# RemoteSensingTools/vSmartMOM.jl

Hardware: AMD Instinct MI355X
Metric: spectral-points/s (whole node) for rt_run, O2-A band (higher is better)
Workload: dtype f64; 1 GPU; C2: O2-A 759-770 nm, nStokes=3, Nquad=20 (N=60), 40 layers, 10000 spectral points/GPU, m=0..2, Rayleigh+synthetic O2 absorption, Lambertian 0.15; ranks=1, collective_backend=none (1 rank), N=60, layers=40, points_per_gpu=10000, fourier_moments=3

## Files before the change

include/vsmartmom_hip.h:

```cpp
#ifndef VSMARTMOM_HIP_H
#define VSMARTMOM_HIP_H

#include <stddef.h>
#include <stdint.h>

#ifdef __cplusplus
extern "C" {
#endif

typedef enum vsm_status {
  VSM_OK = 0,
  VSM_ERR_INVALID_ARG = 1,
  VSM_ERR_UNSUPPORTED = 2,
  VSM_ERR_HIP = 3,
  VSM_ERR_NO_DEVICE = 4
} vsm_status;

typedef enum vsm_iface {
  VSM_IFACE_00 = 0,
  VSM_IFACE_01 = 1,
  VSM_IFACE_10 = 2,
  VSM_IFACE_11 = 3
} vsm_iface;

// ... 387 lines not shown
int vsm_run_create_view_f64(const vsm_quad_f64* q, int S, int nm, const int* m_h, const int* coupling_h, void* workspace,
                            size_t workspace_bytes, unsigned flags, int nrows, const int* rows_h, vsm_run** run);
int vsm_run_create_view_f32(const vsm_quad_f32* q, int S, int nm, const int* m_h, const int* coupling_h, void* workspace,
                            size_t workspace_bytes, unsigned flags, int nrows, const int* rows_h, vsm_run** run);
int vsm_run_layer_f64(vsm_run* run, int ndoubl, const double* dtau, const double* varpi, const double* tau_sum,
                      const double* F0, int ncomp, const double* const* Zpp, const double* const* Zmp, long long z_stride,
                      const double* fcomp, int toa, const int* layer_coupling_h, void* stream);
int vsm_run_layer_f32(vsm_run* run, int ndoubl, const float* dtau, const float* varpi, const float* tau_sum,
                      const float* F0, int ncomp, const float* const* Zpp, const float* const* Zmp, long long z_stride,
                      const float* fcomp, int toa, const int* layer_coupling_h, void* stream);
int vsm_run_export_f64(vsm_run* run, const vsm_composite_f64* comps, void* stream);
int vsm_run_export_f32(vsm_run* run, const vsm_composite_f32* comps, void* stream);
int vsm_run_import_f64(vsm_run* run, const vsm_composite_f64* comps, void* stream);
int vsm_run_import_f32(vsm_run* run, const vsm_composite_f32* comps, void* stream);
int vsm_run_zw_tail(vsm_run* run);
int vsm_run_view_rows(vsm_run* run, int nrows, const int* rows_h);
int vsm_run_view_block(const vsm_run* run, int block, int* im, int* n, int* nv, int* local_rows);
int vsm_run_view_rows(vsm_run* run, int nrows, const int* rows_h);
int vsm_run_view_block(const vsm_run* run, int block, int* im, int* n, int* nv, int* local_rows);
int vsm_run_destroy(vsm_run* run);
enum { VSM_SURFACE_LAMBERTIAN_SCALAR = 0, VSM_SURFACE_LAMBERTIAN_SPECTRAL = 1, VSM_SURFACE_BRDF = 2 };
enum { VSM_SURFACE_LAYER_IDENTITY = 1 };
unsigned vsm_surface_layer_flags(int kind, int m, int has_surface_source);
int vsm_run_export_moment_f64(vsm_run* run, int im, const vsm_composite_f64* comp, void* stream);
int vsm_run_export_moment_f32(vsm_run* run, int im, const vsm_composite_f32* comp, void* stream);
int vsm_run_export_sources_f64(vsm_run* run, int im, const vsm_composite_f64* comp, void* stream);
int vsm_run_export_sources_f32(vsm_run* run, int im, const vsm_composite_f32* comp, void* stream);
int vsm_run_surface_f64(vsm_run* run, int im, int iface, const vsm_added_f64* added_surface, int identity, int matrices,
                        const vsm_composite_f64* comp, double* work, void* stream);
int vsm_run_surface_f32(vsm_run* run, int im, int iface, const vsm_added_f32* added_surface, int identity, int matrices,
                        const vsm_composite_f32* comp, float* work, void* stream);
int vsm_run_guard_once(vsm_run* run);
int vsm_run_counters(const vsm_run* run, int* counts_h);
int vsm_stokes_coupling_f64(int N, int n_stokes, int nblocks, const double* Zpp, const double* Zmp, int* mask_d, void* stream);
int vsm_stokes_coupling_f32(int N, int n_stokes, int nblocks, const float* Zpp, const float* Zmp, int* mask_d, void* stream);

typedef struct vsm_added_rs_f64 {
  double *ier_mp, *iet_pp, *ier_pm, *iet_mm;
  double *ieJ0_p, *ieJ0_m;
  int K;
  int reserved;
} vsm_added_rs_f64;
typedef struct vsm_added_rs_f32 {
  float *ier_mp, *iet_pp, *ier_pm, *iet_mm;
  float *ieJ0_p, *ieJ0_m;
  int K;
  int reserved;
} vsm_added_rs_f32;
typedef struct vsm_composite_rs_f64 {
  double *ieR_mp, *ieR_pm, *ieT_pp, *ieT_mm;
  double *ieJ0_p, *ieJ0_m;
  int K;
  int reserved;
} vsm_composite_rs_f64;
typedef struct vsm_composite_rs_f32 {
  float *ieR_mp, *ieR_pm, *ieT_pp, *ieT_mm;
  float *ieJ0_p, *ieJ0_m;
  int K;
  int reserved;
} vsm_composite_rs_f32;
typedef struct vsm_rrs_f64 {
  const int* shift;
  const double* varpi_ie;
  const double* fscatt;
  const double* Zpp;
  const double* Zmp;
// ... 272 lines not shown
```

vsmartmom.jl_amd/_lib.py:

```python
from __future__ import annotations

import ctypes as C
import os

_HERE = os.path.dirname(os.path.abspath(__file__))
LIB_PATH = os.environ.get("VSM_LIB_PATH") or os.path.join(_HERE, "lib", "libvsmartmom_hip.so")


class VSMError(RuntimeError):
    pass


class vsm_quad_f64(C.Structure):
    _fields_ = [("mu", C.c_void_p), ("wt", C.c_void_p), ("N", C.c_int), ("n_stokes", C.c_int),
                ("i_mu0", C.c_int), ("mu0", C.c_double)]


class vsm_quad_f32(C.Structure):
    _fields_ = [("mu", C.c_void_p), ("wt", C.c_void_p), ("N", C.c_int), ("n_stokes", C.c_int),
                ("i_mu0", C.c_int), ("mu0", C.c_float)]


class vsm_added(C.Structure):
    _fields_ = [("r_mp", C.c_void_p), ("t_pp", C.c_void_p), ("r_pm", C.c_void_p), ("t_mm", C.c_void_p),
# ... 115 lines not shown
    "vsm_interaction_inelastic_rrs_{T}": (_I, [_I, _I, _I, _P, _P, _P, _P, _P, _P, _P]),
    "vsm_copy_added_to_composite_ie_{T}": (_I, [_I, _I, _P, _P, _P]),
    "vsm_postprocess_vza_ie_{T}": (_I, [_I, _I, _I, _I, _I, _P, _P, _P, _P, _P, _P, _P]),
    "vsm_ss_column_{T}": (_I, [_P, _I, _I, _I, _P, _P, _P, _P, _P, _P, _P, _P, _P, _P, _I, _P, _P, _P, _P, _P, _P, _P]),
    "vsm_ss_column_lin_{T}": (_I, [_P, _I, _I, _I, _I, _I, _I, _I, _I, _P, _P, _P, _P, _P, _P, _P, _P, _P, _P, _I, _P, _P, _P, _P, _P, _P, _P,
                                   _P, _P, _I, _P, _P, _P, _P, _P]),
    "vsm_ss_column_rrs_{T}": (_I, [_P, _I, _I, _I, _I, _P, _P, _P, _P, _P, _P, _P, _P, _I, _I, _P, _P, _P, _P, _P]),
    "vsm_ss_column_rrs_lin_{T}": (_I, [_P, _I, _I, _I, _I, _I, _I, _I, _I, _P, _P, _P, _P, _P, _P, _P, _P, _P, _P, _P, _I, _I, _P, _P, _P,
                                       _P, _P]),
    "vsm_exact_ss_path1_{T}": (_I, [_I, _I, _I, _I, _I, _P, _P, _P, _P, "{R}", _P, _P, _P]),
    "vsm_exact_ss_path2_{T}": (_I, [_I, _I, _I, _I, _I, _P, _P, _I, _P, "{R}", _P, _P, _P]),
    "vsm_exact_ss_path34_{T}": (_I, [_I, _I, _I, _I, _I, _P, _P, _P, _P, _P, _P, _P, _P, "{R}", _P, _P, _P, _P]),
    "vsm_exact_ss_jac12_{T}": (_I, [_I, _I, _I, _I, _I, _P, _P, _P, _P, _I, _P, "{R}", _P, _P, _P, _P, _P, _P, _P]),
    "vsm_run_supported": (_I, [_I, _I, _I]),
    "vsm_run_workspace_bytes": (_SZ, [_I, _I, _I, _I, _P]),
    "vsm_run_supported_f32": (_I, [_I, _I, _I]),
    "vsm_run_workspace_bytes_f32": (_SZ, [_I, _I, _I, _I, _P]),
    "vsm_run_create_{T}": (_I, [_P, _I, _I, _P, _P, _P, _SZ, _P]),
    "vsm_run_create_ex_{T}": (_I, [_P, _I, _I, _P, _P, _P, _SZ, C.c_uint, _P]),
    "vsm_run_create_view_{T}": (_I, [_P, _I, _I, _P, _P, _P, _SZ, C.c_uint, _I, _P, _P]),
    "vsm_run_layer_{T}": (_I, [_P, _I, _P, _P, _P, _P, _I, _P, _P, _LL, _P, _I, _P, _P]),
    "vsm_run_export_{T}": (_I, [_P, _P, _P]),
    "vsm_run_import_{T}": (_I, [_P, _P, _P]),
    "vsm_run_zw_tail": (_I, [_P]),
    "vsm_run_view_rows": (_I, [_P, _I, _P]),
    "vsm_run_view_block": (_I, [_P, _I, _P, _P, _P, _P]),
    "vsm_run_destroy": (_I, [_P]),
    "vsm_surface_layer_flags": (C.c_uint, [_I, _I, _I]),
    "vsm_run_export_moment_{T}": (_I, [_P, _I, _P, _P]),
    "vsm_run_export_sources_{T}": (_I, [_P, _I, _P, _P]),
    "vsm_run_surface_{T}": (_I, [_P, _I, _I, _P, _I, _I, _P, _P, _P]),
    "vsm_run_guard_once": (_I, [_P]),
    "vsm_run_counters": (_I, [_P, _P]),
    "vsm_stokes_coupling_{T}": (_I, [_I, _I, _I, _P, _P, _P, _P]),
    "vsm_level_radiance_work_elems": (_SZ, [_I, _I]),
    "vsm_level_radiance_{T}": (_I, [_I, _I, _I, _I, _P, _P, _P, _P, _P, _LL, _P, _P, _P, _P, _P, _P, _P]),
    "vsm_level_radiance_oplevel_{T}": (_I, [_I, _I, _I, _I, _P, _P, _P, _P, _P, _LL, _P, _P, _P, _P, _P, _P, _P]),
    "vsm_level_radiance_src_{T}": (_I, [_I, _I, _I, _I, _P, _P, _P, _I, _P, _P, _LL, _P, _P, _P, _P, _P, _P, _P]),
    "vsm_level_flux_{T}": (_I, [_I, _I, _I, _P, _I, _P, _P, _LL, _P, _I, _P, _P, "{R}", _P, _P, _P, _P]),
    "vsm_surface_emission_response_{T}": (_I, [_I, _I, _I, _I, _P, _I, _P, _P, _P, _P, _P, _LL, _P, _P, _P]),
    "vsm_level_radiance_ie_{T}": (_I, [_I, _I, _I, _I, _P, _I, _P, _P, _P, _P, _LL, _P, _P, _P, _P, _P, _P, _P, _P, _P, _P, _P]),
    "vsm_level_flux_ie_{T}": (_I, [_I, _I, _I, _I, _P, _P, _P, _LL, _P, _P, _P, _P, _P, _P, _I, _P, _P, "{R}", _P, _P, _P, _P]),
    "vsm_level_radiance_lin_{T}": (_I, [_I, _I, _I, _I, _I, _I, _P, _P, _P, _P, _LL, _P, _P, _P, _LL, _P, _P, _LL, _LL, _P, _P, _P, _P, _P,
                                        _P]),
    "vsm_level_radiance_lin_src_{T}": (_I, [_I, _I, _I, _I, _I, _I, _I, _P, _P, _P, _P, _LL, _P, _P, _P, _LL, _P, _P, _LL, _LL, _P, _P, _P,
                                            _P, _P, _P, _P, _P]),
    "vsm_level_flux_lin_{T}": (_I, [_I, _I, _I, _I, _I, _I, _P, _P, _LL, _P, _P, _P, _LL, _P, _P, _LL, _LL, _P, _P, _P, _I, _P, _P,
                                    "{R}", _P, _P, _P, _I, _P, _P]),
    "vsm_mie_work_elems": (_SZ, [_I, _I, _I]),
    "vsm_mie_nai2": (_I, [_I, _I, _I, C.c_double, C.c_double, C.c_double, _P, _P, _P, _P, _P, _P, _P, _P, _P, _P, _P]),
    "vsm_mie_lin_work_elems": (_SZ, [_I, _I, _I]),
    "vsm_mie_nai2_lin": (_I, [_I, _I, _I, C.c_double, C.c_double, C.c_double] + [_P] * 16),
    "vsm_dbge_work_elems": (_SZ, [_I, _I]),
    "vsm_truncate_dbge": (_I, [_I, _I, _I, C.c_double, _P, _P, _P, _P, _P, _P, _P, _P, _P, _P]),
    "vsm_dbge_lin_work_elems": (_SZ, [_I, _I]),
    "vsm_truncate_dbge_lin": (_I, [_I, _I, _I, C.c_double] + [_P] * 15),
    "vsm_absorption_chunk": (_I, []),
    "vsm_absorption_work_elems": (_SZ, [_I, _I]),
    "vsm_absorption_xsec": (_I, [_I, _I, _I, _I] + [_P] * 15 + [C.c_double, C.c_double, _I, _I, _I, _P, _P, _P]),
    "vsm_absorption_lin_chunk": (_I, []),
    "vsm_absorption_lin_work_elems": (_SZ, [_I, _I]),
    "vsm_absorption_xsec_lin": (_I, [_I, _I, _I, _I] + [_P] * 16 + [C.c_double, C.c_double, _I, _I, _I] + [_P] * 6),
    "vsm_absorption_profile_slots": (_I, [_I, _I, _I] + [_P] * 6),
    "vsm_test_lds_mm_{T}": (_I, [_I, _I, _P, _P, _P, _P]),
    "vsm_test_lds_inv_{T}": (_I, [_I, _I, _P, _P, _I, _P, _P]),
    "vsm_test_poison_lds": (_I, [_P]),
# ... 97 lines not shown
```

vsmartmom.jl_amd/core_rt.py:

```python
from __future__ import annotations

import contextlib
import ctypes as C
import dataclasses
import math
import os
import warnings
from dataclasses import dataclass
from typing import List, Optional

import numpy as np
import torch

from . import _lib
from . import host_model as H
from .architectures import GPU, CPU, architecture, array_type, devi, synchronize_if_gpu, to_host

IFACE = {"00": 0, "01": 1, "10": 2, "11": 3}
MOMENT_BATCH = 4
MOMENT_BATCH_MAX = 24
MOMENT_BATCHING = True
THERMAL_FUSION = True
NATIVE_RUN = True
NATIVE_SOURCES_ONLY = True
NATIVE_VIEW_ROWS = True
VIEW_ROWS_MAX = 16
NATIVE_ZW_TAIL = True
NATIVE_IDENTITY_SURFACE = True
NATIVE_DROPIN = True
REFERENCE_ORDER = False


def _require_gpu(arch):
    if not isinstance(arch, GPU):
        raise _lib.VSMError("vsmartmom.jl_amd provides the MI355X path only; architecture %r has no compute path here "
                            "(no CPU fallback by design)" % (arch,))
    if not torch.cuda.is_available():
        raise _lib.VSMError("no MI355X visible to HIP (torch.cuda.is_available() is False)")
    if arch.device_index != torch.cuda.current_device():
        raise _lib.VSMError("architecture GPU(%d) is not the current HIP device (%d): one process per GPU -- call "
                            "torch.cuda.set_device(%d) first" % (arch.device_index, torch.cuda.current_device(),
                                                                 arch.device_index))


def _torch_dtype(FT):
    return torch.float64 if np.dtype(FT) == np.float64 else torch.float32


def _stream_ptr():
    return C.c_void_p(torch.cuda.current_stream().cuda_stream)


def _ptr(t: Optional[torch.Tensor]):
    return C.c_void_p(0 if t is None else t.data_ptr())


def to_device_matrix(A: np.ndarray, arch, FT) -> torch.Tensor:
    A = np.asarray(A, dtype=FT)
    if A.ndim == 2:
        A = A[None]
# ... 68 lines not shown
    def __init__(self, FT, arch, N, nSpec, shared=False, d_symmetric=0):
        dev, dt = devi(arch), _torch_dtype(FT)
        sm = 1 if shared else nSpec
        z = lambda: torch.zeros((sm, N, N), dtype=dt, device=dev)
        self.r_mp, self.t_pp = z(), z()
        self.d_symmetric = int(d_symmetric)
        self.r_pm, self.t_mm = (None, None) if self.d_symmetric else (z(), z())
        self.j0_p = torch.zeros((nSpec, N), dtype=dt, device=dev)
        self.j0_m = torch.zeros((nSpec, N), dtype=dt, device=dev)
        self.N, self.nSpec, self.shared, self.dtype = N, nSpec, shared, dt

    def cstruct(self):
        return _lib.vsm_added(self.r_mp.data_ptr(), self.t_pp.data_ptr(),
                              0 if self.r_pm is None else self.r_pm.data_ptr(),
                              0 if self.t_mm is None else self.t_mm.data_ptr(),
                              self.j0_p.data_ptr(), self.j0_m.data_ptr(), 0 if self.shared else self.N * self.N,
                              self.d_symmetric, 0)


def _composite_field(name):
    vector = name in ("J0_p", "J0_m")

    def fget(self):
        if vector and self._vectors_current:
            return self._arr[name]
        return self.materialize()._arr[name]

    def fset(self, value):
        self.materialize()._arr[name] = value
    return property(fget, fset)


RUN_COUNTERS = ("exports_full", "exports_src", "surface_interactions", "guard_launches")


class RunRef:

    def __init__(self, run, sink=None, keep=None, refs: int = 1):
        self.run, self.sink, self.keep, self.refs = run, sink, keep, refs

    def release(self):
        self.refs -= 1
        if self.refs == 0 and self.run is not None:
            run, self.run = self.run, None
            L = _lib.lib()
            if self.sink is not None:
                counts = (C.c_int * 4)()
                if L.vsm_run_counters(run, counts) == 0:
                    for k, v in zip(RUN_COUNTERS, counts):
                        self.sink[k] = self.sink.get(k, 0) + int(v)
            L.vsm_run_destroy(run)
            self.keep = None


class CompositeLayer:

    def __init__(self, FT, arch, N, nSpec):
        dev, dt = devi(arch), _torch_dtype(FT)
        z = lambda: torch.zeros((nSpec, N, N), dtype=dt, device=dev)
        self._native = None
        self._sources_only = False
        self._view_rows = None
        self._native_ws = None
        self._vectors_current = False
        self._counters = None
        self._arr = dict(R_mp=z(), R_pm=z(), T_pp=z(), T_mm=z(), J0_p=torch.zeros((nSpec, N), dtype=dt, device=dev),
                         J0_m=torch.zeros((nSpec, N), dtype=dt, device=dev))
        self.N, self.nSpec, self.dtype = N, nSpec, dt

    R_mp, R_pm, T_pp = _composite_field("R_mp"), _composite_field("R_pm"), _composite_field("T_pp")
    T_mm, J0_p, J0_m = _composite_field("T_mm"), _composite_field("J0_p"), _composite_field("J0_m")

    def materialize(self):
        slot = self._native
        if slot is None:
            return self
        self._native, self._vectors_current = None, False
        try:
            cc = self._cstruct_raw()
            _lib.call("vsm_run_export_moment", self.dtype, slot.run, slot.im, C.byref(cc), _stream_ptr())
        finally:
            slot.ref.release()
        return self
# ... 785 lines not shown
                    m = mom["m"]
                    weight = float(fourier_weight(FT, m))
                    flags = create_surface_layer_(model.surface, self.added_surface, m, self.dq, mom["tau_sum_surface"], rho=mom["rho"],
                                                  has_surface_source=has_surface_source)
                    if surface_source_contribute_(self, model.surface, self.added_surface, m):
                        flags &= ~SURFACE_LAYER_IDENTITY
                    identity = bool(flags & SURFACE_LAYER_IDENTITY) and NATIVE_IDENTITY_SURFACE and mom["iface_surface"] == "11"
                    if not comp.surface_step(mom["iface_surface"], self.added_surface, identity, streams is not None, self.work):
                        interaction_(mom["iface_surface"], comp, self.added_surface, work=self.work)
                    if self.compute_hdrf:
                        interaction_hdrf_(pol, comp, self.added_surface, m, self.dq, model.vza, model.vaz, self.qp, weight,
                                          self.hdr_J, self.hdr, self.bhr_uw, self.bhr_dw)
                    postprocessing_vza_(pol, comp, model.vza, model.vaz, self.qp, m, weight, self.R_SFI, self.T_SFI)
                    thermal_pass = self.thermal_B is not None and (m == 0 or (m == 1 and self.thermal_slot().carry))
                    if thermal_pass:
                        self._thermal_slot(mom, weight)
                    if streams is not None:
                        Jm, Jp = comp.J0_m.clone(), comp.J0_p.clone()
                        if thermal_pass:
                            Jm += self._thermal.comp.J0_m
                            Jp += self._thermal.comp.J0_p
                        streams.append(dict(m=m, weight=weight, R_mp=comp.R_mp.clone(), T_pp=comp.T_pp.clone(), J0_m=Jm, J0_p=Jp))
        if isinstance(model.surface, H.CoxMunkSurface) and self.ss_correction:
            apply_ss_correction_(self.R_SFI, model.surface, pol, model.vza, model.vaz, self.qp.mu0,
                                 self.moments[-1]["tau_sum_surface"], model.m_max, self.arch, FT)
        return self.R_SFI, self.T_SFI

    def _drop_lazy(self):
        for c in self._composites:
            if c._vectors_current:
                c.drop_native()

    def run_counters(self) -> dict:
        tot = {k: 0 for k in RUN_COUNTERS}
        tot.update(self.__dict__.get("_run_counts", {}))
        live = {id(c._native.ref): c._native.ref for c in self._composites if c._native is not None}
        for ref in live.values():
            counts = (C.c_int * 4)()
            _lib.check(_lib.lib().vsm_run_counters(ref.run, counts))
            for k, v in zip(RUN_COUNTERS, counts):
                tot[k] += int(v)
        return tot

    def _group_size(self, sequential: bool) -> int:
        want = max(MOMENT_BATCH, min(MOMENT_BATCH_MAX, 4096 // max(self.S, 1)))
        return 1 if sequential else min(want, len(self.moments))

    @contextlib.contextmanager
    def _walk_composites(self, nb: int, sources_only: bool, view_rows):
        while len(self._composites) < nb:
            self._composites.append(make_composite_layer(self.FT, self.arch, (self.N, self.N), self.S))
        for c in self._composites:
            c._sources_only = bool(sources_only)
            c._view_rows = view_rows if sources_only else None
            c._counters = self.__dict__.setdefault("_run_counts", {})
        try:
            yield
        finally:
            for c in self._composites:
                c._sources_only = False
                c._view_rows = None

    def _walk_layers(self, group, comps, nat, sources_only: bool, view_rows, trace=None, keep_added: bool = False, tops_at=(),
                     keep_top=None, keep_native: bool = False):
        eps2 = 2 * np.finfo(self.FT).eps
        if nat:
            def export(l):
                def cb(cs):
                    for k, c in zip(nat, cs):
                        keep_top(k, l, (c._arr["R_pm"].clone(), c._arr["J0_p"].clone()))
                return cb
            self._run_layers_native([group[k] for k in nat], [comps[k] for k in nat], sources_only=sources_only,
                                    export_at={l: export(l) for l in tops_at}, view_rows=view_rows, keep_native=keep_native)
        rest = [k for k in range(len(group)) if k not in nat]
# ... 11 lines not shown
                               work=self.work, keep_added=keep_added)
            if iz + 1 in tops_at:
                for k, comp in zip(rest, comps_l):
                    keep_top(k, iz + 1, comp.snapshot_top())

    def _native_moments(self):
        if not NATIVE_RUN or getattr(self, "coupling", None) is None or not self.moments:
            return set()
        eps2 = 2 * np.finfo(self.FT).eps
        for iz, ly in enumerate(self.moments[0]["layers"]):
            p = ly["props"]
            if p.max_tau_varpi <= eps2 or (iz > 0 and ly["iface"] != "11") or (p.fcomp is not None and p.fcomp.shape[1] > 4):
                return set()
        return {i for i, mom in enumerate(self.moments) if run_supported(self.dt, self.N, self.pol.n, int(self.coupling[mom["m"]]))}

    def _run_layers_native(self, group, comps, sources_only: bool = True, export_at=None, view_rows=None, keep_native: bool = False):
        L = _lib.lib()
        self._drop_lazy()
        nm, N, S, ns = len(group), self.N, self.S, self.pol.n
        marr = (C.c_int * nm)(*[int(mom["m"]) for mom in group])
        carr = (C.c_int * nm)(*[int(self.coupling[mom["m"]]) for mom in group])
        nbytes = run_workspace_bytes(self.dt, N, ns, S, nm, carr)
        ws = getattr(self, "_native_ws", None)
        if ws is None or ws.numel() * 8 < nbytes:
            ws = self._native_ws = _lib.poison(torch.empty(max(nbytes // 8, 2), dtype=torch.float64, device=self.dev))
        q = self.dq.cstruct()
        run = C.c_void_p()
        run_create_(self.dt, q, S, nm, marr, carr, ws, nbytes, sources_only, view_rows, run)
        ref = RunRef(run, self.__dict__.setdefault("_run_counts", {}), keep=(ws, self.dq))
        try:
            _lib.check(L.vsm_run_guard_once(run))
            if NATIVE_ZW_TAIL and not torch.cuda.is_current_stream_capturing():
                _lib.check(L.vsm_run_zw_tail(run))
            for iz in range(self.Nz):
                ly0 = group[0]["layers"][iz]
                props = [mom["layers"][iz]["props"] for mom in group]
                p0 = props[0]
                zpp = (C.c_void_p * nm)(*[p.Zpp.data_ptr() for p in props])
                zmp = (C.c_void_p * nm)(*[p.Zmp.data_ptr() for p in props])
                ncomp = 0 if p0.fcomp is None else int(p0.fcomp.shape[1])
                lc = (C.c_int * nm)(*[self._layer_coupling(mom["m"], iz) for mom in group])
                run_layer_native_(run, nm, int(ly0["nd"]), ly0["dtau"], p0.varpi, ly0["tau_sum"], self.F0, ncomp, zpp, zmp,
                                  0 if ncomp else p0.z_stride, p0.fcomp, iz == 0, lc, self.dt)
                if export_at and (iz + 1) in export_at:
                    cc = (type(comps[0].cstruct()) * nm)(*[c.cstruct() for c in comps])
                    _lib.call("vsm_run_export", self.dt, run, cc, _stream_ptr())
                    export_at[iz + 1](comps)
            if keep_native:
                for im, (mom, c) in enumerate(zip(group, comps)):
                    c.drop_native()
                    mask = int(self.coupling[mom["m"]])
                    c._native = NativeSlot(run, int(mom["m"]), mask, stokes_groups(ns, mask), ref, im)
                    ref.refs += 1
            else:
                cc = (type(comps[0].cstruct()) * nm)(*[c.cstruct() for c in comps])
                _lib.call("vsm_run_export", self.dt, run, cc, _stream_ptr())
        finally:
            ref.release()

    def thermal_slot(self) -> "ThermalSlot":
        if self._thermal is None:
            self._thermal = ThermalSlot(self)
        return self._thermal

    def _thermal_slot(self, mom, weight):
        th = self.thermal_slot()
# ... 175 lines not shown
```

vsmartmom.jl_amd/csrc/vsm_elemental.h:

```cpp
#pragma once
#include "vsm_common.h"

namespace vsm {

template <typename T>
__device__ __forceinline__ T expm1_small(T y) {
  T q = T(1.0 / 39916800.0);
  q = fma(q, y, T(1.0 / 3628800.0));
  q = fma(q, y, T(1.0 / 362880.0));
  q = fma(q, y, T(1.0 / 40320.0));
  q = fma(q, y, T(1.0 / 5040.0));
  q = fma(q, y, T(1.0 / 720.0));
  q = fma(q, y, T(1.0 / 120.0));
  q = fma(q, y, T(1.0 / 24.0));
  q = fma(q, y, T(1.0 / 6.0));
  q = fma(q, y, T(0.5));
  q = fma(q, y, T(1.0));
  return q * y;
}
template <typename T>
__device__ __forceinline__ T expdiff_tab_thin(T xi, T xj, T ai, T aj, T ej) {
  const T dlt = xi - xj;
  return (fabs(dlt) > T(0.125) * fmax(xi, xj)) ? (ai - aj) : ej * expm1_small<T>(-dlt);
}
template <typename T>
__device__ __forceinline__ T expdiff_tab_thick(T xi, T xj, T ei, T ej) {
  const T dlt = xi - xj;
  const T v = ((dlt < T(0)) ? ei : ej) * (-expm1(-fabs(dlt)));
  return (dlt < T(0)) ? v : -v;
}

__device__ __forceinline__ double geo_div(double a, double b) { return a / b; }
__device__ __forceinline__ float geo_div(float a, float b) { return __fdividef(a, b); }

template <typename T>
__device__ __forceinline__ void elemental_pair(T w, T zp, T zm, T mi, T xi, T ai, T ei, T mj, T xj, T aj, T ej, T wct, bool diag,
                                               bool thick, T& rr, T& tt) {
  rr = w * zm * geo_div(mj, mi + mj) * wct * (-(ai + aj + ai * aj));
  T ediff;
  if (thick) ediff = expdiff_tab_thick<T>(xi, xj, ei, ej); else ediff = expdiff_tab_thin<T>(xi, xj, ai, aj, ej);
  const T t_off = w * zp * geo_div(mj, mi - mj) * wct * ediff;
  const T t_1 = w * zp * xi * wct;
  const T t_same = diag ? ei * (T(1) + t_1) : ej * t_1;
  tt = (mi == mj) ? t_same : t_off;
}

}
```

vsmartmom.jl_amd/csrc/vsm_native.hip:

```cpp
#include <stdlib.h>

#include <vector>

#include "vsm_native_dev.h"
#include "vsm_native_run.h"

#ifndef VSM_NATIVE_PARK_RT
#define VSM_NATIVE_PARK_RT 3
#endif

namespace vsm {

struct nlayer_comps {
  double* c[NSUB_MAX];
};

namespace {

template <int RT, int KS, int KZ = KS, bool TILE = false>
__device__ __forceinline__ void ned_body(nsmem<RT, (4 * KS + 2 > 16 * RT)>& sm, npos<RT>& p, int n, int gsz, unsigned uvmask, int ndoubl,
                                         const double* __restrict__ img, nstrip<RT>& r_s, nstrip<RT>& t_s, int* status) {
  using G = ngeo<RT>;
  constexpr unsigned dP = 0, dQ = G::AF * 8;
  double* jp = sm.vec[0];
// ... 1153 lines not shown
    }
    R[naf_idx<RT>(i, j)] = rv;
    T[naf_idx<RT>(i, j)] = tv;
  }
  if (ph == 0) {
    const int i0 = ns * q.i_mu0;
    const double mu0n = q.mu[i0];
    const double x0 = d / mu0n, e0 = exp(-x0), a0 = expm1(-x0);
    double zp = 0.0, zm = 0.0;
    for (int qq = 0; qq < ns; ++qq) {
      const long long zo = fi + (long long)N * (i0 + qq);
      const double f = F0[qq + (long long)ns * s];
      zp += zget(Zp, zo) * f;
      zm += zget(Zm, zo) * f;
    }
    double rr, tt;
    elemental_pair(w, zp, zm, mi, xi, ai, ei, mu0n, x0, a0, e0, (m == 0) ? 0.5 : 0.25, false, thick || x0 >= 0.5, rr, tt);
    const double att = exp(-tau_sum[s] / mu0n);
    const double vp = (i < n) ? tt * att : 0.0;
    const double vm = (i < n) ? rr * att * sg : 0.0;
    const double expk0 = exp(-d / q.mu0);
    out[2 * G::AF + i] = vp;
    out[2 * G::AF + NP + i] = vm;
    out[2 * G::AF + 2 * NP + i] = expk0;
    if (riders_in) {
      T[naf_idx<RT>(i, c1)] = vp;
      T[naf_idx<RT>(i, c2)] = vm * expk0;
      R[naf_idx<RT>(i, c1)] = vm;
      R[naf_idx<RT>(i, c2)] = vp;
    }
  }
}

template <typename T>
struct ngroup_map {
  int ngroups;
  int grp_of[4];
  int pos_in[4];
  int gsz[4];
  int rt[4];
  int n[4];
  T* base[4];
};
__device__ __forceinline__ int nat_idx_rt(const double*, int rt, int i, int j) {
  const int w = j >> 4, l15 = j & 15, ta = i >> 4, mm = i & 15, kq = mm & 3, r = mm >> 2;
  const int lane = (kq << 4) | l15, u = 2 * ta + (r >> 1);
  return ((w * 2 * rt + u) * 64 + lane) * 2 + (r & 1);
}
__device__ __forceinline__ int nat_idx_rt(const float*, int rt, int i, int j) {
  const int w = j >> 4, l15 = j & 15, ta = i >> 4, mm = i & 15, kq = mm & 3, r = mm >> 2;
  return ((w * rt + ta) * 64 + ((kq << 4) | l15)) * 4 + r;
}
__device__ __forceinline__ void nat_elem_rt(const double*, int rt, int e, int& i, int& j) {
  const int half = e & 1, lane = (e >> 1) & 63, unit = (e >> 7) % (2 * rt), w = (e >> 7) / (2 * rt);
  i = 16 * (unit >> 1) + (lane >> 4) + 4 * (2 * (unit & 1) + half), j = 16 * w + (lane & 15);
}
__device__ __forceinline__ void nat_elem_rt(const float*, int rt, int e, int& i, int& j) {
  const int r = e & 3, lane = (e >> 2) & 63, ta = (e >> 8) % rt, w = (e >> 8) / rt;
  i = 16 * ta + (lane >> 4) + 4 * r, j = 16 * w + (lane & 15);
}
template <typename T>
__global__ __launch_bounds__(256) void k_native_export(int N, int ns, int src, int view, ngroup_map<T> gm, nview vw, composite<T> c) {
  const int s = blockIdx.x, tid = threadIdx.x;
  const long long NN = (long long)N * N;
  T* out[4] = {c.R_mp + s * NN, c.R_pm + s * NN, c.T_pp + s * NN, c.T_mm + s * NN};
  for (int e = tid; e < N * N; e += 256) {
// ... 287 lines not shown
#define VSM_NI(KS) \
  case KS: return VSM_NCAT(launch_ia_native_, KS)(N, S, c, a, status, st);
  switch ((N + 3) / 4) {
    VSM_NI(1) VSM_NI(2) VSM_NI(3) VSM_NI(4) VSM_NI(5) VSM_NI(6) VSM_NI(7) VSM_NI(8) VSM_NI(9) VSM_NI(10) VSM_NI(11) VSM_NI(12)
    VSM_NI(13) VSM_NI(14) VSM_NI(15) VSM_NI(16)
    default: break;
  }
#undef VSM_NI
  return VSM_ERR_UNSUPPORTED;
}
namespace {

template <int RT>
static void launch_pre(bool mix, const quad<double>& q, int S, int nsub, int n, int ndoubl, const double* dtau, const double* varpi,
                       const double* tau_sum, const double* F0, const npre_args<double>& a, double* pre, hipStream_t st) {
  const dim3 grid(S, nsub), block(64 * RT);
  if (mix)
    hipLaunchKernelGGL((k_elemental_native<RT, true>), grid, block, 0, st, q, n, ndoubl, dtau, varpi, tau_sum, F0, a, pre);
  else
    hipLaunchKernelGGL((k_elemental_native<RT, false>), grid, block, 0, st, q, n, ndoubl, dtau, varpi, tau_sum, F0, a, pre);
}

static void native_launch_pre(int rt, bool mix, const quad<double>& q, int S, int nsub, int n, int ndoubl, const double* dtau,
                              const double* varpi, const double* tau_sum, const double* F0, const npre_args<double>& a, double* pre,
                              hipStream_t st) {
  switch (rt) {
    case 1: launch_pre<1>(mix, q, S, nsub, n, ndoubl, dtau, varpi, tau_sum, F0, a, pre, st); break;
    case 2: launch_pre<2>(mix, q, S, nsub, n, ndoubl, dtau, varpi, tau_sum, F0, a, pre, st); break;
    case 3: launch_pre<3>(mix, q, S, nsub, n, ndoubl, dtau, varpi, tau_sum, F0, a, pre, st); break;
    case 4: launch_pre<4>(mix, q, S, nsub, n, ndoubl, dtau, varpi, tau_sum, F0, a, pre, st); break;
    case 5: launch_pre<5>(mix, q, S, nsub, n, ndoubl, dtau, varpi, tau_sum, F0, a, pre, st); break;
    default: launch_pre<6>(mix, q, S, nsub, n, ndoubl, dtau, varpi, tau_sum, F0, a, pre, st); break;
  }
}
static void native_launch_pre(int rt, bool mix, const quad<float>& q, int S, int nsub, int n, int ndoubl, const float* dtau,
                              const float* varpi, const float* tau_sum, const float* F0, const npre_args<float>& a, float* pre,
                              hipStream_t st) {
  native32_launch_pre(rt, mix, q, S, nsub, n, ndoubl, dtau, varpi, tau_sum, F0, a, pre, st);
}
static int native_launch_layer(const nat_sub& h, int S, int nsub, int ndoubl, int toa, int src, const double* pre, double* const* comps,
                               int* status, const nview* vw, hipStream_t st) {
  return launch_layer_native(h.ks, h.ks - h.kz, S, nsub, h.n, h.uvmask, h.gsz, ndoubl, toa, src, pre, comps, status, vw, st);
}
static int native_launch_layer(const nat_sub& h, int S, int nsub, int ndoubl, int toa, int, const float* pre, float* const* comps,
                               int* status, const nview*, hipStream_t st) {
  return native32_launch_layer(h.ks, S, nsub, h.n, h.uvmask, h.gsz, ndoubl, toa, pre, comps, status, st);
}

template <typename T>
static ngroup_map<T> group_map(const vsm_run* run, int im) {
  ngroup_map<T> gm;
  gm.ngroups = 0;
  for (int a = 0; a < 4; ++a) {
    gm.grp_of[a] = gm.pos_in[a] = 0;
    gm.gsz[a] = gm.rt[a] = 1;
    gm.n[a] = 0;
    gm.base[a] = nullptr;
  }
  for (const nat_sub& sb : run->subs) {
    if (sb.im != im) continue;
    const int g = gm.ngroups++;
    gm.gsz[g] = sb.gsz;
    gm.rt[g] = sb.rt;
    gm.n[g] = sb.n;
    gm.base[g] = static_cast<T*>(run->ws) + sb.comp_off;
    for (int k = 0; k < sb.gsz; ++k) {
// ... 201 lines not shown
      } else {
        triv[run->pure_diag[i] ? 2 : 0].push_back(i);
      }
    }
    for (int mode = 0; mode < 3; ++mode) {
      if (triv[mode].empty()) continue;
      ndiag_args<T> da;
      const int nt = (int)triv[mode].size();
      for (int k = 0; k < NSUB_MAX; ++k) {
        const nat_sub& sb = run->subs[triv[mode][k < nt ? k : 0]];
        da.comp[k] = ws + sb.comp_off;
        da.gsz[k] = sb.gsz;
        da.g0[k] = sb.g[0] | (sb.g[1] << 4) | (sb.g[2] << 8) | (sb.g[3] << 12);
      }
      hipLaunchKernelGGL((k_native_diag_layer<T>), dim3(run->S, nt), dim3(256), 0, st, q, h.rt, h.n, (T)ldexp(1.0, ndoubl), mode,
                         src, view, dtau, da, view ? view_of(run, triv[mode]) : nview{});
      VSM_LAUNCH_CHECK("k_native_diag_layer");
    }
    const int nsub = (int)act.size();
    if (!nsub) continue;
    npre_args<T> pa;
    T* lc[NSUB_MAX];
    for (int k = 0; k < NSUB_MAX; ++k) {
      const nat_sub& sb = run->subs[act[k < nsub ? k : 0]];
      pa.s[k].m = sb.m;
      pa.s[k].gsz = sb.gsz;
      for (int a = 0; a < 4; ++a) pa.s[k].g[a] = sb.g[a];
      VSM_REQUIRE(Zpp[sb.im] && Zmp[sb.im], "vsm_run_layer: null Z of moment %d", sb.im);
      pa.s[k].z = zsrc<T>{Zpp[sb.im], Zmp[sb.im], ncomp ? 0 : z_stride, ncomp, fcomp};
      lc[k] = ws + sb.comp_off;
    }
    T* pre_cl = pre + off;
    off += pre_stride_rt(h.rt) * (size_t)run->S * nsub;
    native_launch_pre(h.rt, ncomp > 0, q, run->S, nsub, h.n, ndoubl, dtau, varpi, tau_sum, F0, pa, pre_cl, st);
    VSM_LAUNCH_CHECK("k_elemental_native");
    const nview vw = view ? view_of(run, act) : nview{};
    const int rc = native_launch_layer(h, run->S, nsub, ndoubl, toa, src, pre_cl, lc, status, view ? &vw : nullptr, st);
    if (rc) return rc;
  }
  return VSM_OK;
}

template <typename T, typename CS, bool IMPORT>
static int run_convert(vsm_run* run, const CS* comps, void* stream) {
  VSM_REQUIRE(run && comps, "vsm_run_export / import: null argument");
  VSM_REQUIRE(run->elem_size == (int)sizeof(T), "vsm_run_export / import: the run was created for %d-byte arrays", run->elem_size);
  if (IMPORT) ++run->imports;
  if (run->S == 0) return VSM_OK;
  if (IMPORT) {
    run->pure_diag.assign(run->subs.size(), 0);
    run->flags &= ~(unsigned)VSM_RUN_ZW_TAIL;
    for (nat_sub& sb : run->subs) sb.kz = sb.ks;
    run->guard_once = false;
  }
  for (int im = 0; im < run->nm; ++im) {
    const CS& c = comps[im];
    VSM_REQUIRE(c.R_mp && c.R_pm && c.T_pp && c.T_mm && c.J0_p && c.J0_m, "vsm_run_export / import: null composite array (moment %d)", im);
    const composite<T> cc{c.R_mp, c.R_pm, c.T_pp, c.T_mm, c.J0_p, c.J0_m};
    const ngroup_map<T> gm = group_map<T>(run, im);
    const int view = (run->flags & VSM_RUN_VIEW_ROWS) ? 1 : 0;
    const nview vw = view ? view_of_moment(run, im) : nview{};
    if (IMPORT)
      hipLaunchKernelGGL((k_native_import<T>), dim3(run->S), dim3(256), 0, as_stream(stream), run->N, run->ns, view, gm, vw, cc);
    else
      hipLaunchKernelGGL((k_native_export<T>), dim3(run->S), dim3(256), 0, as_stream(stream), run->N, run->ns,
                         (run->flags & VSM_RUN_SOURCES_ONLY) ? 1 : 0, view, gm, vw, cc);
    VSM_LAUNCH_CHECK("k_native_export / import");
    if (!IMPORT) ++run->exports_full;
// ... 173 lines not shown
}
int vsm_run_export_sources_f64(vsm_run* run, int im, const vsm_composite_f64* comp, void* stream) {
  return run_export_moment<double>(run, im, comp, false, stream, "vsm_run_export_sources");
}
int vsm_run_export_sources_f32(vsm_run* run, int im, const vsm_composite_f32* comp, void* stream) {
  return run_export_moment<float>(run, im, comp, false, stream, "vsm_run_export_sources");
}

int vsm_run_surface_f64(vsm_run* run, int im, int iface, const vsm_added_f64* added_surface, int identity, int matrices,
                        const vsm_composite_f64* comp, double* work, void* stream) {
  return run_surface<double>(run, im, iface, added_surface, identity, matrices, comp, work, stream, vsm_interaction_f64);
}
int vsm_run_surface_f32(vsm_run* run, int im, int iface, const vsm_added_f32* added_surface, int identity, int matrices,
                        const vsm_composite_f32* comp, float* work, void* stream) {
  return run_surface<float>(run, im, iface, added_surface, identity, matrices, comp, work, stream, vsm_interaction_f32);
}

int vsm_run_guard_once(vsm_run* run) {
  VSM_REQUIRE(run, "vsm_run_guard_once: null argument");
  VSM_REQUIRE(run->layers == 0 && run->imports == 0, "vsm_run_guard_once: the run has taken layer steps or an import already");
  run->guard_once = true;
  return VSM_OK;
}

int vsm_run_counters(const vsm_run* run, int* counts) {
  VSM_REQUIRE(run && counts, "vsm_run_counters: null argument");
  counts[0] = run->exports_full;
  counts[1] = run->exports_src;
  counts[2] = run->surface_ia;
  counts[3] = run->guards;
  return VSM_OK;
}

int vsm_stokes_coupling_f64(int N, int n_stokes, int nblocks, const double* Zpp, const double* Zmp, int* mask_d, void* stream) {
  return stokes_coupling<double>(N, n_stokes, nblocks, Zpp, Zmp, mask_d, stream);
}
int vsm_stokes_coupling_f32(int N, int n_stokes, int nblocks, const float* Zpp, const float* Zmp, int* mask_d, void* stream) {
  return stokes_coupling<float>(N, n_stokes, nblocks, Zpp, Zmp, mask_d, stream);
}

}

#endif
```

vsmartmom.jl_amd/csrc/vsm_native_run.h:

```cpp
#pragma once
#include <vector>

#include "vsm_internal.h"

namespace vsm {

constexpr int NSUB_MAX = VSM_MM_MAX;

struct nat_sub {
  int im;
  int m;
  int gsz, g[4];
  unsigned uvmask;
  int n, rt, ks;
  int kz;
  size_t comp_off;
  int nv;
  int vrow[VSM_RUN_VIEW_MAX];
};

struct nview {
  int nv[NSUB_MAX];
  unsigned pk[NSUB_MAX][VSM_RUN_VIEW_MAX / 4];
  __host__ __device__ int row(int k, int v) const { return (int)((pk[k][v >> 2] >> (8 * (v & 3))) & 255u); }
  __host__ __device__ int find(int k, int r) const {
    int at = -1;
    for (int v = 0; v < nv[k]; ++v) at = row(k, v) == r ? v : at;
    return at;
  }
};

}

struct vsm_run {
  const void *mu, *wt;
  int N, ns, i_mu0;
  double mu0;
  int elem_size;
  int S, nm;
  unsigned flags;
  std::vector<int> view_rows;
  std::vector<int> m;
  std::vector<vsm::nat_sub> subs;
  std::vector<std::vector<int>> classes;
  void* ws;
  size_t ws_elems;
  int layers = 0;
  int imports = 0;
  std::vector<char> pure_diag;
  bool guard_once = false;
  int exports_full = 0, exports_src = 0, surface_ia = 0, guards = 0;
};

namespace vsm {

constexpr int NATIVE_MAX_ROWS = 96;
constexpr int NATIVE32_MAX_ROWS = 128;

constexpr int rt_of(int n) {
  const int ks = (n + 3) / 4;
  return (ks % 4 == 0 && ks >= 4) ? ks / 4 : (4 * ks + 2 + 15) / 16;
}
constexpr size_t comp_stride_rt(int rt) { return (size_t)4 * (16 * rt) * (16 * rt) + 2 * 16 * rt; }
constexpr size_t pre_stride_rt(int rt) { return (size_t)2 * (16 * rt) * (16 * rt) + 3 * 16 * rt; }

template <typename T>
struct nsub_pre {
  int m, gsz;
  int g[4];
  zsrc<T> z;
};
template <typename T>
struct npre_args {
  nsub_pre<T> s[NSUB_MAX];
};

void native32_launch_pre(int rt, bool mix, const quad<float>& q, int S, int nsub, int n, int ndoubl, const float* dtau,
                         const float* varpi, const float* tau_sum, const float* F0, const npre_args<float>& a, float* pre,
                         hipStream_t st);
int native32_launch_layer(int ks, int S, int nsub, int n, unsigned uvmask, int gsz, int ndoubl, int toa, const float* pre,
                          float* const* comps, int* status, hipStream_t st);

}
```

Baseline: 27060 spectral-points/s.

## Compute elemental layer geometry per quadrature node pair instead of per matrix element

Adds a node-level elemental prepass kernel that computes the geometric factors (mu ratios, exponential differences) once per quadrature node pair in LDS and then assembles the R/T elemental matrices per Stokes row from those shared factors. It is enabled when all Stokes components of a node share the same mu, which is checked once on the host at run setup. This removes redundant exp/divide work repeated ns^2 times per node pair in the f64 elemental kernel. The cost is extra LDS usage, a host memcpy at setup, and a second code path that must match the original arithmetic.

```diff
diff --git a/include/vsmartmom_hip.h b/include/vsmartmom_hip.h
--- a/include/vsmartmom_hip.h
+++ b/include/vsmartmom_hip.h
@@ -443,6 +443,8 @@
                         const vsm_composite_f32* comp, float* work, void* stream);
 int vsm_run_guard_once(vsm_run* run);
 int vsm_run_counters(const vsm_run* run, int* counts_h);
+int vsm_run_node_prepass(vsm_run* run);
+int vsm_run_prepass_counters(const vsm_run* run, int* counts_h);
 int vsm_stokes_coupling_f64(int N, int n_stokes, int nblocks, const double* Zpp, const double* Zmp, int* mask_d, void* stream);
 int vsm_stokes_coupling_f32(int N, int n_stokes, int nblocks, const float* Zpp, const float* Zmp, int* mask_d, void* stream);
 
diff --git a/vsmartmom.jl_amd/_lib.py b/vsmartmom.jl_amd/_lib.py
--- a/vsmartmom.jl_amd/_lib.py
+++ b/vsmartmom.jl_amd/_lib.py
@@ -171,6 +171,8 @@
     "vsm_run_surface_{T}": (_I, [_P, _I, _I, _P, _I, _I, _P, _P, _P]),
     "vsm_run_guard_once": (_I, [_P]),
     "vsm_run_counters": (_I, [_P, _P]),
+    "vsm_run_node_prepass": (_I, [_P]),
+    "vsm_run_prepass_counters": (_I, [_P, _P]),
     "vsm_stokes_coupling_{T}": (_I, [_I, _I, _I, _P, _P, _P, _P]),
     "vsm_level_radiance_work_elems": (_SZ, [_I, _I]),
     "vsm_level_radiance_{T}": (_I, [_I, _I, _I, _I, _P, _P, _P, _P, _P, _LL, _P, _P, _P, _P, _P, _P, _P]),
diff --git a/vsmartmom.jl_amd/core_rt.py b/vsmartmom.jl_amd/core_rt.py
--- a/vsmartmom.jl_amd/core_rt.py
+++ b/vsmartmom.jl_amd/core_rt.py
@@ -26,6 +26,7 @@
 NATIVE_VIEW_ROWS = True
 VIEW_ROWS_MAX = 16
 NATIVE_ZW_TAIL = True
+NATIVE_NODE_PREPASS = True
 NATIVE_IDENTITY_SURFACE = True
 NATIVE_DROPIN = True
 REFERENCE_ORDER = False
@@ -160,6 +161,16 @@
 
 
 RUN_COUNTERS = ("exports_full", "exports_src", "surface_interactions", "guard_launches")
+PREPASS_COUNTERS = ("prepass_elements", "prepass_nodes")
+
+
+def _add_run_counts(L, run, tot):
+    counts, pre = (C.c_int * 4)(), (C.c_int * 2)()
+    rc = L.vsm_run_counters(run, counts) or L.vsm_run_prepass_counters(run, pre)
+    if rc == 0:
+        for k, v in zip(RUN_COUNTERS + PREPASS_COUNTERS, list(counts) + list(pre)):
+            tot[k] = tot.get(k, 0) + int(v)
+    return rc
 
 
 class RunRef:
@@ -173,10 +184,7 @@
             run, self.run = self.run, None
             L = _lib.lib()
             if self.sink is not None:
-                counts = (C.c_int * 4)()
-                if L.vsm_run_counters(run, counts) == 0:
-                    for k, v in zip(RUN_COUNTERS, counts):
-                        self.sink[k] = self.sink.get(k, 0) + int(v)
+                _add_run_counts(L, run, self.sink)
             L.vsm_run_destroy(run)
             self.keep = None
 
@@ -1028,14 +1036,17 @@
                 c.drop_native()
 
     def run_counters(self) -> dict:
-        tot = {k: 0 for k in RUN_COUNTERS}
+        return {k: v for k, v in self._all_run_counts().items() if k in RUN_COUNTERS}
+
+    def prepass_counters(self) -> dict:
+        return {k: v for k, v in self._all_run_counts().items() if k in PREPASS_COUNTERS}
+
+    def _all_run_counts(self) -> dict:
+        tot = {k: 0 for k in RUN_COUNTERS + PREPASS_COUNTERS}
         tot.update(self.__dict__.get("_run_counts", {}))
         live = {id(c._native.ref): c._native.ref for c in self._composites if c._native is not None}
         for ref in live.values():
-            counts = (C.c_int * 4)()
-            _lib.check(_lib.lib().vsm_run_counters(ref.run, counts))
-            for k, v in zip(RUN_COUNTERS, counts):
-                tot[k] += int(v)
+            _lib.check(_add_run_counts(_lib.lib(), ref.run, tot))
         return tot
 
     def _group_size(self, sequential: bool) -> int:
@@ -1113,6 +1124,8 @@
             _lib.check(L.vsm_run_guard_once(run))
             if NATIVE_ZW_TAIL and not torch.cuda.is_current_stream_capturing():
                 _lib.check(L.vsm_run_zw_tail(run))
+            if NATIVE_NODE_PREPASS and not torch.cuda.is_current_stream_capturing():
+                _lib.check(L.vsm_run_node_prepass(run))
             for iz in range(self.Nz):
                 ly0 = group[0]["layers"][iz]
                 props = [mom["layers"][iz]["props"] for mom in group]
diff --git a/vsmartmom.jl_amd/csrc/vsm_elemental.h b/vsmartmom.jl_amd/csrc/vsm_elemental.h
--- a/vsmartmom.jl_amd/csrc/vsm_elemental.h
+++ b/vsmartmom.jl_amd/csrc/vsm_elemental.h
@@ -45,4 +45,31 @@
   tt = (mi == mj) ? t_same : t_off;
 }
 
+template <typename T>
+struct node_pair {
+  T gm, fac, gp, ed;
+};
+template <typename T>
+__device__ __forceinline__ node_pair<T> elemental_node_pair(T mi, T xi, T ai, T ei, T mj, T xj, T aj, T ej, bool thick) {
+#pragma clang fp contract(off)
+  node_pair<T> f;
+  f.gm = geo_div(mj, mi + mj);
+  f.fac = -fma(ai, aj, ai + aj);
+  if (mi == mj) {
+    f.gp = xi;
+    f.ed = ej;
+  } else {
+    f.gp = geo_div(mj, mi - mj);
+    if (thick) f.ed = expdiff_tab_thick<T>(xi, xj, ei, ej); else f.ed = expdiff_tab_thin<T>(xi, xj, ai, aj, ej);
+  }
+  return f;
 }
+template <typename T>
+__device__ __forceinline__ void elemental_assemble(T w, T zp, T zm, T wct, bool diag, const node_pair<T>& f, T& rr, T& tt) {
+#pragma clang fp contract(off)
+  rr = w * zm * f.gm * wct * f.fac;
+  const T p = w * zp * f.gp;
+  tt = f.ed * (diag ? fma(p, wct, T(1)) : p * wct);
+}
+
+}
diff --git a/vsmartmom.jl_amd/csrc/vsm_native.hip b/vsmartmom.jl_amd/csrc/vsm_native.hip
--- a/vsmartmom.jl_amd/csrc/vsm_native.hip
+++ b/vsmartmom.jl_amd/csrc/vsm_native.hip
@@ -1209,6 +1209,148 @@
   }
 }
 
+constexpr int NODE_PRE_MAX = 32;
+inline size_t node_pre_lds(int nn) { return (size_t)(nn * nn + nn) * sizeof(node_pair<double>); }
+
+template <int RT>
+__global__ __launch_bounds__(64 * RT) void k_elemental_nodes(quad<double> q, int n, int nsub, int ndoubl, const double* __restrict__ dtau,
+                                                             const double* __restrict__ varpi, const double* __restrict__ tau_sum,
+                                                             const double* __restrict__ F0, npre_args<double> a,
+                                                             double* __restrict__ pre) {
+  using G = ngeo<RT>;
+  constexpr int NP = G::NP, NT = G::NT;
+  extern __shared__ __attribute__((aligned(16))) unsigned char node_raw[];
+  node_pair<double>* pt = reinterpret_cast<node_pair<double>*>(node_raw);
+  __shared__ double mus[NODE_PRE_MAX], xs[NODE_PRE_MAX], es[NODE_PRE_MAX], ems[NODE_PRE_MAX];
+  __shared__ double wcts[NP];
+  __shared__ int frow[NP], node_of[NP];
+  __shared__ int thick_flag;
+  const int s = blockIdx.x, tid = threadIdx.x;
+  const int N = q.N, ns = q.n_stokes, gsz = a.s[0].gsz;
+  const int nn = (n + gsz - 1) / gsz;
+  const double d = dtau[s], w = varpi[s];
+  if (tid < nn) {
+    const double mu = q.mu[tid * ns + a.s[0].g[0]];
+    const double x = d / mu;
+    mus[tid] = mu;
+    xs[tid] = x;
+    es[tid] = exp(-x);
+    ems[tid] = expm1(-x);
+  }
+  if (tid < NP) node_of[tid] = min(tid, n - 1) / gsz;
+  if (tid == 0) thick_flag = 0;
+  __syncthreads();
+  if (tid < nn && xs[tid] >= 0.5) thick_flag = 1;
+  __syncthreads();
+  const bool thick = thick_flag != 0;
+  const int i0s = ns * q.i_mu0;
+  const double mu0n = q.mu[i0s];
+  for (int p = tid; p < nn * nn + nn; p += NT) {
+    if (p < nn * nn) {
+      const int ni = p / nn, nj = p - ni * nn;
+      pt[p] = elemental_node_pair(mus[ni], xs[ni], ems[ni], es[ni], mus[nj], xs[nj], ems[nj], es[nj], thick);
+    } else {
+      const int ni = p - nn * nn;
+      const double x0 = d / mu0n, e0 = exp(-x0), a0 = expm1(-x0);
+      pt[p] = elemental_node_pair(mus[ni], xs[ni], ems[ni], es[ni], mu0n, x0, a0, e0, thick || x0 >= 0.5);
+    }
+  }
+  const int rp = tid % (NP / 2), ph = tid / (NP / 2);
+  const int ta = rp >> 3, m0 = (rp & 7) << 1;
+  const int ia = 16 * ta + m0, ib = ia + 1;
+  const int na = node_of[ia], nb = node_of[ib];
+  const int Kend = ((n + 3) >> 2) << 2;
+  const int c1 = Kend, c2 = Kend + 1;
+  const bool riders_in = ndoubl > 0 && c2 < NP;
+  double att = 0.0, expk0 = 0.0;
+  if (tid < NP) {
+    att = exp(-tau_sum[s] / mu0n);
+    expk0 = exp(-d / q.mu0);
+  }
+  for (int k = 0; k < nsub; ++k) {
+    const nsub_pre<double>& sp = a.s[k];
+    const int m = sp.m;
+    const double* Zp = sp.z.Zpp + (long long)s * sp.z.zs;
+    const double* Zm = sp.z.Zmp + (long long)s * sp.z.zs;
+    __syncthreads();
+    if (tid < NP) {
+      const bool in = tid < n;
+      const int fr = in ? (tid / gsz) * ns + sp.g[tid % gsz] : 0;
+      const double wt = in ? q.wt[fr] : 0.0;
+      frow[tid] = fr;
+      wcts[tid] = (m == 0) ? wt / 2.0 : wt / 4.0;
+    }
+    __syncthreads();
+    double* out = pre + ((long long)k * gridDim.x + s) * G::PRE_STRIDE;
+    double* R = out;
+    double* T = out + G::AF;
+    const bool uva = ia < n && sp.g[ia % gsz] >= 2, uvb = ib < n && sp.g[ib % gsz] >= 2;
+    const double sga = (ndoubl >= 1 && uva) ? -1.0 : 1.0, sgb = (ndoubl >= 1 && uvb) ? -1.0 : 1.0;
+    const int fa = frow[min(ia, n - 1)], fb = frow[min(ib, n - 1)];
+    for (int j = ph; j < NP; j += 8) {
+      if (riders_in && (j == c1 || j == c2)) continue;
+      double ra = 0.0, rb = 0.0, tA = 0.0, tB = 0.0;
+      if (j < n) {
+        const double wct = wcts[j];
+        if (wct > num<double>::eps()) {
+          const int nj = node_of[j];
+          const long long zc = (long long)N * frow[j];
+          if (ia < n) {
+            const node_pair<double> f = pt[na * nn + nj];
+            double rr, tt;
+            elemental_assemble(w, Zp[fa + zc], Zm[fa + zc], wct, ia == j, f, rr, tt);
+            ra = rr * sga;
+            tA = tt;
+          }
+          if (ib < n) {
+            const node_pair<double> f = pt[nb * nn + nj];
+            double rr, tt;
+            elemental_assemble(w, Zp[fb + zc], Zm[fb + zc], wct, ib == j, f, rr, tt);
+            rb = rr * sgb;
+            tB = tt;
+          }
+        } else {
+          if (ia == j) tA = es[na];
+          if (ib == j) tB = es[nb];
+        }
+      }
+      const int ks = j >> 2, kk = j & 3, sw = kk | ((ks & 3) << 2);
+      const int at = (ks * RT + ta) * 64 + ((kk << 4) | ((m0 ^ sw) & 14));
+      const bool swp = sw & 1;
+      *reinterpret_cast<nd2_t*>(R + at) = nd2_t{swp ? rb : ra, swp ? ra : rb};
+      *reinterpret_cast<nd2_t*>(T + at) = nd2_t{swp ? tB : tA, swp ? tA : tB};
+    }
+    if (tid < NP) {
+      const int i = tid;
+      double vp = 0.0, vm = 0.0;
+      if (i < n) {
+        const int fi = frow[i];
+        double zp = 0.0, zm = 0.0;
+        for (int qq = 0; qq < ns; ++qq) {
+          const long long zo = fi + (long long)N * (i0s + qq);
+          const double f = F0[qq + (long long)ns * s];
+          zp = fma(Zp[zo], f, zp);
+          zm = fma(Zm[zo], f, zm);
+        }
+        const double sg = (ndoubl >= 1 && sp.g[i % gsz] >= 2) ? -1.0 : 1.0;
+        double rr, tt;
+        elemental_assemble(w, zp, zm, (m == 0) ? 0.5 : 0.25, false, pt[nn * nn + node_of[i]], rr, tt);
+        vp = tt * att;
+        vm = rr * att * sg;
+      }
+      out[2 * G::AF + i] = vp;
+      out[2 * G::AF + NP + i] = vm;
+      out[2 * G::AF + 2 * NP + i] = expk0;
+      if (riders_in) {
+        T[naf_idx<RT>(i, c1)] = vp;
+        T[naf_idx<RT>(i, c2)] = vm * expk0;
+        R[naf_idx<RT>(i, c1)] = vm;
+        R[naf_idx<RT>(i, c2)] = vp;
+      }
+    }
+  }
+}
+
 template <typename T>
 struct ngroup_map {
   int ngroups;
@@ -1562,6 +1704,31 @@
     case 5: launch_pre<5>(mix, q, S, nsub, n, ndoubl, dtau, varpi, tau_sum, F0, a, pre, st); break;
     default: launch_pre<6>(mix, q, S, nsub, n, ndoubl, dtau, varpi, tau_sum, F0, a, pre, st); break;
   }
+}
+template <int RT>
+static void launch_pre_nodes(const quad<double>& q, int S, int nsub, int n, int nn, int ndoubl, const double* dtau, const double* varpi,
+                             const double* tau_sum, const double* F0, const npre_args<double>& a, double* pre, hipStream_t st) {
+  hipLaunchKernelGGL((k_elemental_nodes<RT>), dim3(S), dim3(64 * RT), node_pre_lds(nn), st, q, n, nsub, ndoubl, dtau, varpi, tau_sum,
+                     F0, a, pre);
+}
+static bool native_launch_pre_nodes(const vsm_run* run, const nat_sub& h, int ncomp, const quad<double>& q, int nsub, int ndoubl,
+                                    const double* dtau, const double* varpi, const double* tau_sum, const double* F0,
+                                    const npre_args<double>& a, double* pre, hipStream_t st) {
+  const int nn = (h.n + h.gsz - 1) / h.gsz;
+  if (!run->node_prepass || ncomp > 0 || nn > NODE_PRE_MAX) return false;
+  switch (h.rt) {
+    case 1: launch_pre_nodes<1>(q, run->S, nsub, h.n, nn, ndoubl, dtau, varpi, tau_sum, F0, a, pre, st); break;
+    case 2: launch_pre_nodes<2>(q, run->S, nsub, h.n, nn, ndoubl, dtau, varpi, tau_sum, F0, a, pre, st); break;
+    case 3: launch_pre_nodes<3>(q, run->S, nsub, h.n, nn, ndoubl, dtau, varpi, tau_sum, F0, a, pre, st); break;
+    case 4: launch_pre_nodes<4>(q, run->S, nsub, h.n, nn, ndoubl, dtau, varpi, tau_sum, F0, a, pre, st); break;
+    case 5: launch_pre_nodes<5>(q, run->S, nsub, h.n, nn, ndoubl, dtau, varpi, tau_sum, F0, a, pre, st); break;
+    default: launch_pre_nodes<6>(q, run->S, nsub, h.n, nn, ndoubl, dtau, varpi, tau_sum, F0, a, pre, st); break;
+  }
+  return true;
+}
+static bool native_launch_pre_nodes(const vsm_run*, const nat_sub&, int, const quad<float>&, int, int, const float*, const float*,
+                                    const float*, const float*, const npre_args<float>&, float*, hipStream_t) {
+  return false;
 }
 static void native_launch_pre(int rt, bool mix, const quad<float>& q, int S, int nsub, int n, int ndoubl, const float* dtau,
                               const float* varpi, const float* tau_sum, const float* F0, const npre_args<float>& a, float* pre,
@@ -1829,8 +1996,14 @@
     }
     T* pre_cl = pre + off;
     off += pre_stride_rt(h.rt) * (size_t)run->S * nsub;
-    native_launch_pre(h.rt, ncomp > 0, q, run->S, nsub, h.n, ndoubl, dtau, varpi, tau_sum, F0, pa, pre_cl, st);
-    VSM_LAUNCH_CHECK("k_elemental_native");
+    if (native_launch_pre_nodes(run, h, ncomp, q, nsub, ndoubl, dtau, varpi, tau_sum, F0, pa, pre_cl, st)) {
+      VSM_LAUNCH_CHECK("k_elemental_nodes");
+      run->pre_nodes += nsub;
+    } else {
+      native_launch_pre(h.rt, ncomp > 0, q, run->S, nsub, h.n, ndoubl, dtau, varpi, tau_sum, F0, pa, pre_cl, st);
+      VSM_LAUNCH_CHECK("k_elemental_native");
+      run->pre_image += nsub;
+    }
     const nview vw = view ? view_of(run, act) : nview{};
     const int rc = native_launch_layer(h, run->S, nsub, ndoubl, toa, src, pre_cl, lc, status, view ? &vw : nullptr, st);
     if (rc) return rc;
@@ -2070,6 +2243,25 @@
   return VSM_OK;
 }
 
+int vsm_run_node_prepass(vsm_run* run) {
+  VSM_REQUIRE(run, "vsm_run_node_prepass: null argument");
+  VSM_REQUIRE(run->layers == 0, "vsm_run_node_prepass: the run has taken layer steps already");
+  if (run->elem_size != 8) return VSM_OK;
+  std::vector<double> mu((size_t)run->N);
+  VSM_HIP(hipMemcpy(mu.data(), run->mu, sizeof(double) * (size_t)run->N, hipMemcpyDefault));
+  bool same = true;
+  for (int i = 0; i < run->N; ++i) same = same && mu[(size_t)i] == mu[(size_t)(i / run->ns) * run->ns];
+  run->node_prepass = same;
+  return VSM_OK;
+}
+
+int vsm_run_prepass_counters(const vsm_run* run, int* counts) {
+  VSM_REQUIRE(run && counts, "vsm_run_prepass_counters: null argument");
+  counts[0] = run->pre_image;
+  counts[1] = run->pre_nodes;
+  return VSM_OK;
+}
+
 int vsm_stokes_coupling_f64(int N, int n_stokes, int nblocks, const double* Zpp, const double* Zmp, int* mask_d, void* stream) {
   return stokes_coupling<double>(N, n_stokes, nblocks, Zpp, Zmp, mask_d, stream);
 }
diff --git a/vsmartmom.jl_amd/csrc/vsm_native_run.h b/vsmartmom.jl_amd/csrc/vsm_native_run.h
--- a/vsmartmom.jl_amd/csrc/vsm_native_run.h
+++ b/vsmartmom.jl_amd/csrc/vsm_native_run.h
@@ -50,6 +50,8 @@
   std::vector<char> pure_diag;
   bool guard_once = false;
   int exports_full = 0, exports_src = 0, surface_ia = 0, guards = 0;
+  bool node_prepass = false;
+  int pre_image = 0, pre_nodes = 0;
 };
 
 namespace vsm {
```

New measurement: 27110 spectral-points/s, median of 6. No clear change (+0.2%).
